# nolanderc/gpu-voxel-raytracer

Hardware: AMD Instinct MI355X
Metric: Mrays/s (higher is better)
Workload: dtype f32

## Files before the change

### gpu_voxel_raytracer_amd/csrc/api_context.hip

```cpp
#include <chrono>
#include <memory>

#include "ctx.h"

namespace vxrt {

size_t image_bytes(const vxrt_ctx* c) { return size_t(c->band.local_rows) * c->band.width * sizeof(float4); }
size_t display_bytes(const vxrt_ctx* c) { return size_t(c->band.local_rows) * c->band.width * 4u; }
bool is_display(vxrt_image which) { return which == VXRT_DISPLAY_BGRA8_SRGB || which == VXRT_DISPLAY_RGBA8_SRGB; }

int count_local_rows(const BandMap& b) {
    int rows = 0;
    for (int gb = b.rank; gb < band_count(b); gb += b.nranks) {
        const int y0 = band_first_row(b, gb), n = band_nominal_rows(b, gb);
        rows += (y0 + n <= b.height) ? n : b.height - y0;
    }
    return rows;
}

int local_band_count(const BandMap& b) {
    const int bands = band_count(b);
    return bands <= b.rank ? 0 : (bands - b.rank + b.nranks - 1) / b.nranks;
}

void free_images(vxrt_ctx* c) {
    c->ring.clear();
    c->ring_arena.reset();
    free_halo(c);
    for (DeviceBuf<float4>* p : {&c->accum[0], &c->accum[1], &c->denoised, &c->spp_sum}) p->reset();
    c->display.reset();
    c->schedules.clear();
    c->queues.clear();
    c->queue_bytes = 0;
    c->first_hits.clear();
}

int alloc_images(vxrt_ctx* c) {
    free_images(c);
    size_t bytes = image_bytes(c);
    if (bytes == 0) bytes = sizeof(float4);
    if (size_t(c->band.local_rows) * size_t(c->band.width) >= (size_t(1) << kPixBits)) {
        set_error("more than 2^27 pixels per context");
        return VXRT_E_INVALID;
    }
    c->ring.resize(size_t(c->inflight) * size_t(c->batch) + 2);
    const size_t pitch = (bytes + (size_t(2) << 20) - 1) & ~((size_t(2) << 20) - 1);
    HIP_TRY(c->ring_arena.alloc(pitch * 3 * c->ring.size()));
    HIP_TRY(hipMemsetAsync(c->ring_arena, 0, pitch * 3 * c->ring.size(), c->stream));
    size_t piece = 0;
// ... 36 lines not shown
                char* p = sq.rq_block;
                sq.rq.state[0] = reinterpret_cast<float4*>(p); p += kSegments * cap * 64;
                sq.rq.state[1] = reinterpret_cast<float4*>(p); p += kSegments * cap * 64;
                sq.rq.rays[0] = reinterpret_cast<float4*>(p); p += kSegments * cap * 64;
                sq.rq.rays[1] = reinterpret_cast<float4*>(p); p += kSegments * cap * 64;
                sq.rq.results[0] = reinterpret_cast<uint4*>(p); p += kSegments * cap * 32;
                sq.rq.results[1] = reinterpret_cast<uint4*>(p); p += kSegments * cap * 32;
                sq.rq.counts = reinterpret_cast<unsigned*>(p);
                sq.rq.seg_capacity = unsigned(cap);
            }
        }
    }
    if (c->batch >= 2 && c->band.local_rows > 0) {
        c->first_hits.resize(size_t(c->inflight));
        for (DeviceBuf<uint4>& p : c->first_hits) HIP_TRY(p.alloc(size_t(c->band.local_rows) * size_t(c->band.width)));
    }
    const size_t tiles = trace_tile_count(c->band.width, c->band.local_rows);
    c->schedules.resize(size_t(c->inflight));
    for (vxrt_ctx::TileSchedule& t : c->schedules) {
        for (DeviceBuf<uint32_t>* p : {&t.cost, &t.order, &t.last_cost}) {
            HIP_TRY(p->alloc(tiles + 1));
            HIP_TRY(hipMemsetAsync(p->get(), 0, (tiles + 1) * sizeof(uint32_t), c->stream));
        }
        HIP_TRY(t.scratch.alloc(256 * 128));
        if (c->trace_priority) {
            HIP_TRY(t.host_heavy.alloc(64 / sizeof(unsigned)));
            t.host_heavy[0] = 0u;
            HIP_TRY(t.heavy_ready.create(hipEventDisableTiming));
        }
    }
// ... 156 lines not shown
            return VXRT_OK;
        case VXRT_OPT_TAIL_CAPACITY:
            if (at_create) { c->tail_capacity_override = int(value > 0x7fffffffu ? 0x7fffffffu : value); return VXRT_OK; }
            if (c->trace_variant < 4) return VXRT_OK;
            c->tail_capacity_override = int(value > 0x7fffffffu ? 0x7fffffffu : value);
            return resize_tail_queues(c, value == 0 ? (c->shard_capacity_max / 8u < 4096u ? 4096u : c->shard_capacity_max / 8u) : value);
        case VXRT_OPT_SKY_CULL:
            if (value > 1) { set_error("sky cull must be 0 or 1"); return VXRT_E_INVALID; }
            c->sky_cull = int(value);
            return VXRT_OK;
        case VXRT_OPT_FRAME_LANES:
            if (value > 1) { set_error("frame lanes must be 0 or 1"); return VXRT_E_INVALID; }
            c->frame_lanes = int(value);
            return VXRT_OK;
        case VXRT_OPT_SHARED_PRIMARY:
            if (value > 1) { set_error("shared primary must be 0 or 1"); return VXRT_E_INVALID; }
            c->shared_primary = int(value);
            return VXRT_OK;
        case VXRT_OPT_HALO_ROWS:
            if (value > 4096) { set_error("halo rows must be 0..4096"); return VXRT_E_INVALID; }
            c->halo_min_rows = value;
            return VXRT_OK;
        case VXRT_OPT_TILE_ORDER:
            if (value > 1) { set_error("tile order must be 0 (raster) or 1 (longest first)"); return VXRT_E_INVALID; }
            c->use_tile_order = int(value);
            return VXRT_OK;
        case VXRT_OPT_TILE_SPREAD:
            if (value > 256 && value != VXRT_TILE_SPREAD_AUTO) { set_error("tile spread must be 0..256 or VXRT_TILE_SPREAD_AUTO"); return VXRT_E_INVALID; }
            c->spread_override = value == VXRT_TILE_SPREAD_AUTO ? -1 : int(value);
            return VXRT_OK;
        case VXRT_OPT_TRACE_BLOCKS:
// ... 443 lines not shown
    out->queue_overflow_paths = c->queue_overflow_paths;
    return VXRT_OK;
} VXRT_CATCH

int vxrt_reset_stats(vxrt_ctx* c) try {
    if (!valid_ctx(c)) return VXRT_E_INVALID;
    if (int rc = vxrt_sync(c)) return rc;
    HIP_TRY(hipMemsetAsync(c->d_rays, 0, kRaySlots * 64, c->stream));
    HIP_TRY(hipStreamSynchronize(c->stream));
    c->frames = c->pixels = c->timed_frames = c->timed_launches = 0;
    c->queue_overflow_paths = 0;
    c->ms[0] = c->ms[1] = c->ms[2] = c->ms[3] = c->ms[4] = 0.0;
    c->halo_exchanges = 0;
    c->frame_lane_launches = 0;
    c->shared_primary_launches = 0;
    c->split_launches = 0;
    return VXRT_OK;
} VXRT_CATCH


}
```

### gpu_voxel_raytracer_amd/csrc/api_debug.hip

```cpp
#include "../../include/vxrt_bluenoise.h"
#include "ctx.h"

extern "C" {

int vxrt_debug_tile_costs(vxrt_ctx* c, uint32_t* out, size_t n) try {
    if (!valid_ctx(c) || !out) { set_error("null argument"); return VXRT_E_INVALID; }
    const size_t out_x = size_t((c->band.width + 15) / 16), out_y = size_t((c->band.local_rows + 15) / 16);
    if (n != out_x * out_y || c->schedules.empty()) { set_error("tile count mismatch"); return VXRT_E_INVALID; }
    HIP_TRY(hipSetDevice(c->cfg.device));
    if (int rc = sync_all(c)) return rc;
    int tw = 16, th = 16;
    trace_tile_dims(&tw, &th);
    const size_t kx = size_t((c->band.width + tw - 1) / tw), ky = size_t((c->band.local_rows + th - 1) / th);
    std::vector<uint32_t> raw(kx * ky);
    HIP_TRY(hipMemcpy(raw.data(), c->schedules[size_t(c->last_schedule)].last_cost, raw.size() * sizeof(uint32_t), hipMemcpyDeviceToHost));
    for (size_t i = 0; i < n; i++) out[i] = 0;
    for (size_t y = 0; y < ky; y++)
        for (size_t x = 0; x < kx; x++) {
            uint32_t& o = out[(y * size_t(th) / 16) * out_x + x * size_t(tw) / 16];
            o = raw[y * kx + x] > o ? raw[y * kx + x] : o;
        }
    return VXRT_OK;
} VXRT_CATCH

// ... 117 lines not shown
    return VXRT_OK;
} VXRT_CATCH

int vxrt_debug_culled_pixels(vxrt_ctx* c, uint64_t* count) try {
    if (!valid_ctx(c) || !count) { set_error("null argument"); return VXRT_E_INVALID; }
    if (!c->has_scene) { set_error("no scene set"); return VXRT_E_NOSCENE; }
    HIP_TRY(hipSetDevice(c->cfg.device));
    if (int rc = vxrt_sync(c)) return rc;
    const Cam keep_cam = c->cam, keep_old = c->old_cam;
    const vxrt_uniforms keep_u = c->uniforms;
    update_bindings(c);
    TraceArgs a{};
    frame_constants(c, a);
    a.cam = c->cam;
    a.batch = 1;
    set_cull(c, a, &a.cam, 1);
    c->cam = keep_cam; c->old_cam = keep_old; c->uniforms = keep_u;
    ScratchBuffer b;
    HIP_TRY(b.alloc(sizeof(unsigned long long)));
    HIP_TRY(hipMemsetAsync(b.as<unsigned long long>(), 0, sizeof(unsigned long long), c->stream));
    HIP_TRY(launch_count_culled(a, b.as<unsigned long long>(), c->stream));
    HIP_TRY(hipStreamSynchronize(c->stream));
    unsigned long long n = 0;
    HIP_TRY(hipMemcpy(&n, b.as<unsigned long long>(), sizeof n, hipMemcpyDeviceToHost));
    *count = n;
    return VXRT_OK;
} VXRT_CATCH

int vxrt_debug_shared_primary_launches(vxrt_ctx* c, uint64_t* count) try {
    if (!valid_ctx(c) || !count) { set_error("null argument"); return VXRT_E_INVALID; }
    *count = c->shared_primary_launches;
    return VXRT_OK;
} VXRT_CATCH

int vxrt_debug_dda_rays(vxrt_ctx* c, const float* origins, const float* dirs, size_t n, uint32_t flags, float margin_scale, uint32_t max_steps,
                        float* out_walk, float* out_dda, double ms[4]) try {
    if (!valid_ctx(c) || !origins || !dirs || !out_dda || !ms || (!out_walk && !(flags & 4u))) { set_error("null argument"); return VXRT_E_INVALID; }
#if !VXRT_VARIANTS
    set_error("the DDA prototype is not in this build of libvxrt (compile with -DVXRT_VARIANTS=1)");
    return VXRT_E_INVALID;
#else
    if (!c->has_scene) { set_error("no scene set"); return VXRT_E_NOSCENE; }
    const int levels = int(c->depth) + 1;
    if (levels < 3 || levels > 12) { set_error("the DDA grid wants a tree of depth 2..11 (4 .. 4096 cells per axis)"); return VXRT_E_INVALID; }
    if (n == 0) return VXRT_OK;
    HIP_TRY(hipSetDevice(c->cfg.device));
// ... 176 lines not shown
```

### gpu_voxel_raytracer_amd/csrc/api_frame.hip

```cpp
#include "ctx.h"

namespace vxrt {

int check_render(vxrt_ctx* c, uint32_t flags) {
    if (!valid_ctx(c)) return VXRT_E_INVALID;
    const uint32_t stages = VXRT_ALL | VXRT_DENOISE_INTERIOR | VXRT_DENOISE_EDGE;
    if ((flags & stages) == 0) { set_error("no stage selected"); return VXRT_E_INVALID; }
    if ((flags & VXRT_DENOISE) && (flags & (VXRT_DENOISE_INTERIOR | VXRT_DENOISE_EDGE))) {
        set_error("VXRT_DENOISE is the whole stage: it does not combine with VXRT_DENOISE_INTERIOR / VXRT_DENOISE_EDGE");
        return VXRT_E_INVALID;
    }
    if (!c->has_scene) { set_error("vxrt_render before any scene was set"); return VXRT_E_NOSCENE; }
    const bool window = c->band.nranks > 1 && c->denoise.radius > 0;
    const bool any_denoise = (flags & (VXRT_DENOISE | VXRT_DENOISE_INTERIOR | VXRT_DENOISE_EDGE)) != 0;
    const bool reads_halo = (flags & (VXRT_DENOISE | VXRT_DENOISE_EDGE)) != 0;
    if (any_denoise && window && c->band.band_rows % 16 != 0) {
        set_error("denoise with radius > 0 on row bands needs band_rows to be a multiple of 16 (its 16x16 tiles must not straddle bands)");
        return VXRT_E_INVALID;
    }
    if (reads_halo && window && (flags & (VXRT_TRACE | VXRT_TEMPORAL))) {
        set_error("multi-rank denoise with radius > 0 needs the halo: render TRACE|TEMPORAL, exchange, then DENOISE (or DENOISE_INTERIOR "
                  "while the messages travel and DENOISE_EDGE after vxrt_halo_unpack)");
        return VXRT_E_INVALID;
    }
// ... 101 lines not shown
    if (post) {
        HIP_TRY(hipEventRecord(cur.own, c->stream));
        cur.last_use = cur.own;
        cur.last_use_recorded = true;
    }
    return VXRT_OK;
}

}

extern "C" {

int vxrt_render(vxrt_ctx* c, uint32_t flags) try {
    if (int rc = check_render(c, flags)) return rc;
    HIP_TRY(hipSetDevice(c->cfg.device));
    const bool timed = (flags & VXRT_TIMED) != 0;
    if (flags & VXRT_TRACE) {
        int slot = 0;
        Cam cam, old;
        if (int rc = trace_frames(c, 1, timed, &slot, &cam, &old)) return rc;
    }
    if (int rc = post_stages(c, flags, timed)) return rc;
    if (flags & VXRT_TRACE) c->old_cam_valid = true;
    return VXRT_OK;
} VXRT_CATCH

static int render_sequence(vxrt_ctx* c, uint32_t flags, uint32_t count, const float (*path_pos)[3], const float (*path_dir)[3]) {
    const bool timed = (flags & VXRT_TIMED) != 0;
    const uint32_t batch = (flags & VXRT_TRACE) && batches_frames(c->trace_variant) ? uint32_t(c->batch) : 1u;
    if (batch <= 1) {
// ... 14 lines not shown
        for (uint32_t k = 0; k < g; k++) {
            c->slot = slots[k];
            c->cam = cams[k];
            c->old_cam = olds[k];
            if (int rc = post_stages(c, flags, timed)) return rc;
            c->old_cam_valid = true;
        }
        done += g;
    }
    return VXRT_OK;
}

int vxrt_render_frames(vxrt_ctx* c, uint32_t flags, uint32_t count) try {
    if (int rc = check_render(c, flags)) return rc;
    HIP_TRY(hipSetDevice(c->cfg.device));
    return render_sequence(c, flags, count, nullptr, nullptr);
} VXRT_CATCH

int vxrt_render_path(vxrt_ctx* c, uint32_t flags, uint32_t count, const float (*positions)[3], const float (*directions)[3], float fov) try {
    if (int rc = check_render(c, flags)) return rc;
    if (!positions || !directions) { set_error("null argument"); return VXRT_E_INVALID; }
    HIP_TRY(hipSetDevice(c->cfg.device));
    c->cam_fov = fov;
    return render_sequence(c, flags, count, positions, directions);
} VXRT_CATCH

int vxrt_render_spp(vxrt_ctx* c, uint32_t flags, uint32_t spp) try {
    if (int rc = check_render(c, flags)) return rc;
    if (!(flags & VXRT_TRACE) || spp == 0 || spp > 4096) { set_error("vxrt_render_spp needs VXRT_TRACE and 1 <= spp <= 4096"); return VXRT_E_INVALID; }
    HIP_TRY(hipSetDevice(c->cfg.device));
    const bool timed = (flags & VXRT_TIMED) != 0;
    const size_t pixels = size_t(c->band.local_rows) * c->band.width;
    if (spp > 1 && c->spp_sum == nullptr && pixels > 0) HIP_TRY(c->spp_sum.alloc(pixels));
    const uint32_t batch = batches_frames(c->trace_variant) ? uint32_t(c->batch) : 1u;
    Cam first_old{};
    for (uint32_t done = 0; done < spp;) {
        const uint32_t g = spp - done < batch ? spp - done : batch;
        int slots[kMaxBatch];
        Cam cams[kMaxBatch], olds[kMaxBatch];
        const uint32_t gbuf = done + g == spp ? 1u << (g - 1u) : 0u;
        if (int rc = trace_frames(c, g, timed, slots, cams, olds, nullptr, nullptr, gbuf)) return rc;
        if (done == 0) first_old = olds[0];
        if (spp > 1 && pixels > 0) {
            SppArgs a{};
            for (uint32_t k = 0; k < g; k++) {
// ... 30 lines not shown
```

### gpu_voxel_raytracer_amd/csrc/api_trace.hip

```cpp
#include <algorithm>
#include <cmath>

#include "ctx.h"
#include "vx_vec.h"

namespace vxrt {

int resize_tail_queues(vxrt_ctx* c, unsigned want) {
    want = want > c->shard_capacity_max ? c->shard_capacity_max : (want + 63u) / 64u * 64u;
    if (want == c->shard_capacity) return VXRT_OK;
    if (int rc = sync_all(c)) return rc;
    const size_t new_bytes = (size_t(want) * 64 + 1) * 64, old_bytes = (size_t(c->shard_capacity) * 64 + 1) * 64;
    std::vector<DeviceBuf<float4>> fresh;
    for (vxrt_ctx::StreamQueues& q : c->queues)
        for (DeviceBuf<float4>& p : q.hitq)
            if (p) {
                fresh.emplace_back();
                if (hipError_t e = fresh.back().alloc(new_bytes / sizeof(float4)); e != hipSuccess) return hip_fail(e, "hipMalloc (tail queues)");
            }
    size_t k = 0;
    for (vxrt_ctx::StreamQueues& q : c->queues)
        for (DeviceBuf<float4>& p : q.hitq)
            if (p) {
                p.swap(fresh[k++]);
// ... 62 lines not shown
#endif
    f3 sun_dir = mk3(vx_cos(u.sun_yaw) * vx_cos(u.sun_pitch), -vx_sin(u.sun_pitch), vx_sin(u.sun_yaw) * vx_cos(u.sun_pitch));
    f3 sun_n = norm3(sun_dir), neg_sun_n = norm3(-sun_dir);
    f3 sun_color = u.sun_strength * mk3(u.sun_color[0], u.sun_color[1], u.sun_color[2]);
    a.sun_dir[0] = sun_dir.x; a.sun_dir[1] = sun_dir.y; a.sun_dir[2] = sun_dir.z;
    a.sun_dir_n[0] = sun_n.x; a.sun_dir_n[1] = sun_n.y; a.sun_dir_n[2] = sun_n.z;
    a.neg_sun_dir_n[0] = neg_sun_n.x; a.neg_sun_dir_n[1] = neg_sun_n.y; a.neg_sun_dir_n[2] = neg_sun_n.z;
    a.sun_color[0] = sun_color.x; a.sun_color[1] = sun_color.y; a.sun_color[2] = sun_color.z;
    a.sky_color[0] = u.sky_color[0]; a.sky_color[1] = u.sky_color[1]; a.sky_color[2] = u.sky_color[2];
    a.sun_exponent = 1.0f / (u.sun_size * u.sun_size);
    a.sun_zero_below = 0.0f;
    if (a.sun_exponent > 1.0f && a.sun_exponent < 1e6f) a.sun_zero_below = float(exp(-88.0 / double(a.sun_exponent)) * (1.0 - 1e-4));
    a.sun_size = u.sun_size; a.sun_strength = u.sun_strength; a.emit_strength = u.emit_strength; a.specularity = u.specularity;
}

void set_cull(const vxrt_ctx* c, TraceArgs& a, const Cam* cams, uint32_t g) {
    a.cull = 0;
    if (c->sky_cull && c->box_valid) {
        float far = 0.0f;
        bool sane = true;
        for (uint32_t k = 0; k < g; k++)
            for (int i = 0; i < 3; i++) {
                const float v = fabsf(cams[k].o[i]);
                sane = sane && v < 1e6f && std::isfinite(cams[k].r[i]) && std::isfinite(cams[k].u[i]) && std::isfinite(cams[k].f[i]);
                far = v > far ? v : far;
            }
        if (sane) {
            const float m = 0.01f + ldexpf(far + 2.0f * c->root_size, -16);
            for (int i = 0; i < 3; i++) { a.cull_min[i] = c->box_min[i] - m; a.cull_max[i] = c->box_max[i] + m; }
            a.cull = 1;
        }
    }
}

static int xcd_affine_order(vxrt_ctx* c, vxrt_ctx::TileSchedule& sched, hipStream_t ts) {
    const unsigned tiles = trace_tile_count(c->band.width, c->band.local_rows);
    int tw = 8, th = 8;
    trace_tile_dims(&tw, &th);
    const unsigned tx = unsigned(c->band.width + tw - 1) / unsigned(tw), ty = tiles / (tx ? tx : 1u);
    const unsigned S = unsigned(c->xcd_affinity);
    std::vector<uint32_t> cost(tiles), order;
    order.reserve(tiles);
    HIP_TRY(hipStreamSynchronize(ts));
    HIP_TRY(hipMemcpy(cost.data(), sched.cost, size_t(tiles) * 4, hipMemcpyDeviceToHost));
    const unsigned sx = (tx + S - 1) / S, sy = (ty + S - 1) / S;
    std::vector<unsigned long long> scost(size_t(sx) * sy, 0ull);
    for (unsigned t = 0; t < tiles; t++)
// ... 42 lines not shown
}


struct CountSets {
    unsigned* sets[3] = {nullptr, nullptr, nullptr};
    unsigned J = 0;
    CountSets() = default;
    explicit CountSets(const vxrt_ctx::StreamQueues& sq) : sets{sq.counts3, sq.counts3 + 64 * 16, sq.counts3 + 2 * 64 * 16}, J(sq.launches) {}
    unsigned* read() const { return sets[J % 3]; }
    unsigned* written() const { return sets[(J + 1) % 3]; }
    unsigned* cleared() const { return sets[(J + 2) % 3]; }
};

struct TraceLaunch {
    vxrt_ctx* c; hipStream_t ts; size_t lane; uint32_t g; const int* slots;
    TracePlan plan{};
    TraceArgs a;
    CountSets counts;
    TraceLaunch(vxrt_ctx* c_, hipStream_t ts_, size_t lane_, uint32_t g_, const int* slots_) : c(c_), ts(ts_), lane(lane_), g(g_), slots(slots_) {}
};

static float path_motion_px(const vxrt_ctx* c, uint32_t g, uint32_t F, const float (*path_pos)[3], const float (*path_dir)[3]) {
    const float f_px = 0.5f * float(c->cfg.height) / tanf(0.5f * c->cam_fov);
    float worst = 0.0f;
    for (uint32_t k = 0; k + F <= g; k += F) {
        const float* p0 = path_pos[k]; const float* p1 = path_pos[k + F - 1];
        const float* d0 = path_dir[k]; const float* d1 = path_dir[k + F - 1];
        const float n0 = sqrtf(d0[0] * d0[0] + d0[1] * d0[1] + d0[2] * d0[2]), n1 = sqrtf(d1[0] * d1[0] + d1[1] * d1[1] + d1[2] * d1[2]);
        float cosang = (d0[0] * d1[0] + d0[1] * d1[1] + d0[2] * d1[2]) / (n0 * n1);
        cosang = cosang > 1.0f ? 1.0f : (cosang < -1.0f ? -1.0f : cosang);
        const float ang = acosf(cosang);
        const float dp = sqrtf((p1[0] - p0[0]) * (p1[0] - p0[0]) + (p1[1] - p0[1]) * (p1[1] - p0[1]) + (p1[2] - p0[2]) * (p1[2] - p0[2]));
        float dist = sqrtf((p0[0] - c->root_center[0]) * (p0[0] - c->root_center[0]) + (p0[1] - c->root_center[1]) * (p0[1] - c->root_center[1]) +
                           (p0[2] - c->root_center[2]) * (p0[2] - c->root_center[2]));
        dist = dist < 0.05f * c->root_size ? 0.05f * c->root_size : dist;
        const float px = f_px * (ang > dp / dist ? ang : dp / dist);
        worst = !(px <= worst) ? px : worst;
    }
    return worst;
}

static void plan_trace(TracePlan& p, const vxrt_ctx* c, uint32_t g, const Cam* cams, const float (*path_pos)[3], const float (*path_dir)[3], size_t lane) {
    const bool wide = use_wide(c);
    const vxrt_ctx::TileSchedule& sched = c->schedules[lane];
    const bool ordered = c->use_tile_order && sched.valid;
    const unsigned tiles = trace_tile_count(c->band.width, c->band.local_rows);
    p.hbm = c->svo_count * sizeof(SvoRecord) + c->leaf_count * sizeof(int32_t) > kInfinityCacheBytes;
    p.tracer = (c->auto_tracer && (p.hbm || (g == 1 && c->inflight == 1))) ? 0 : c->trace_variant;
    p.wide_head = wide && (p.tracer == 0 || p.tracer == 4);
    p.wide_tail = wide;
    p.single_tail_launch = p.tracer == 4;
    for (int k = c->tail_from + 1; p.single_tail_launch && k < int(c->cfg.max_bounces); k++)
        if (c->queues[lane].hitq[1] && ((c->tail_split >> k) & 1u)) p.single_tail_launch = false;
    const bool fused = c->fused_tail && p.single_tail_launch && !wide && !p.hbm && c->tail_from < int(c->cfg.max_bounces);
    p.path = p.tracer == 0 ? TracePath::all_in_one : p.tracer == 2 ? TracePath::wavefront : p.tracer < 4 ? TracePath::ray_queue :
             fused ? TracePath::fused : p.tracer == 5 ? TracePath::head_paths : TracePath::head_bounces;
    const bool trace_kernel_head = p.path == TracePath::all_in_one || p.path == TracePath::head_bounces || p.path == TracePath::head_paths;
    p.frame_lanes = (c->frame_lanes && !wide && !p.hbm) ? (g % 8u == 0u ? 8 : (g % 4u == 0u ? 4 : 0)) : 0;
    if (p.frame_lanes && path_pos != nullptr && !(path_motion_px(c, g, uint32_t(p.frame_lanes), path_pos, path_dir) <= 16.0f)) p.frame_lanes = 0;
    p.share = trace_kernel_head && c->shared_primary && g >= 2 && lane < c->first_hits.size() && c->first_hits[lane] != nullptr && !wide && !p.hbm;
    for (uint32_t k = 1; p.share && k < g; k++) p.share = memcmp(&cams[k], &cams[0], sizeof(Cam)) == 0;
    if (p.path == TracePath::head_bounces && c->long_tiles_permille > 0 && ordered && p.tracer == 4 && !wide && !p.hbm) {
        const unsigned n = unsigned((unsigned long long)tiles * c->long_tiles_permille / 1000u);
        p.long_blocks = (n < 1u ? 1u : (n >= tiles ? tiles - 1u : n)) * g;
    }
    if (trace_kernel_head && c->trace_priority && ordered && !sched.heavy_pending && p.long_blocks == 0u && sched.heavy < tiles) p.split_heavy = sched.heavy;
    if (batches_frames(p.tracer) && c->use_tile_order && (!sched.valid || sched.age >= 8))
        p.sort = (c->xcd_affinity > 0 && g == 1 && p.hbm) ? TileSort::xcd_affine : TileSort::longest_first;
}

static void next_frames(vxrt_ctx* c, uint32_t g, int* slots, Cam* cams, Cam* olds, const float (*path_pos)[3], const float (*path_dir)[3]) {
    for (uint32_t k = 0; k < g; k++) {
        if (path_pos) {
            memcpy(c->cam_pos, path_pos[k], sizeof c->cam_pos);
            memcpy(c->cam_dir, path_dir[k], sizeof c->cam_dir);
        }
// ... 34 lines not shown
static void fill_trace_args(TraceLaunch& L, const Cam* cams, uint32_t gbuf_frames, uint32_t first_frame_number) {
    const vxrt_ctx* c = L.c;
    TraceArgs& a = L.a;
    const uint32_t g = L.g;
    const vxrt_ctx::TileSchedule& sched = c->schedules[L.lane];
    frame_constants(c, a);
    for (uint32_t k = 0; k < g; k++) {
        const vxrt_ctx::Slot& sl = c->ring[size_t(L.slots[k])];
        a.out[k] = FrameOut{sl.sampled_color, sl.nd, sl.albedo};
        a.cams[k] = cams[k];
    }
    a.out_color = a.out[0].color; a.out_nd = a.out[0].nd; a.out_albedo = a.out[0].albedo;
    a.batch = int(g);
    a.gbuf_frames = gbuf_frames;
    a.frame_lanes = L.plan.frame_lanes;
    set_cull(c, a, cams, g);
    a.ray_counter = c->d_rays;
    a.tile_order = (c->use_tile_order && sched.valid) ? sched.order : nullptr;
    a.tile_cost = c->use_tile_order ? sched.cost : nullptr;
    a.frame_number = first_frame_number;
    a.cam = cams[0];
    a.tail = PathQueue{nullptr, nullptr, 0};
    a.tail_zero = nullptr;
    a.tail_from = 0;
    if (L.plan.tracer != 0) L.counts = CountSets(c->queues[L.lane]);
    if (L.plan.tracer >= 4) {
        a.tail = PathQueue{c->queues[L.lane].hitq[0], L.counts.written(), c->shard_capacity};
        a.tail_zero = L.counts.cleared();
        a.tail_from = c->tail_from;
    }
}
// ... 32 lines not shown
        HIP_TRY(c->aux_streams[lane].create(hipStreamNonBlocking));
        HIP_TRY(c->aux_fork[lane].create(hipEventDisableTiming));
        HIP_TRY(c->aux_join[lane].create(hipEventDisableTiming));
    }
    TraceArgs al = L.a;
    al.tail = PathQueue{nullptr, nullptr, 0};
    al.tail_zero = nullptr;
    HIP_TRY(hipEventRecord(c->aux_fork[lane], L.ts));
    HIP_TRY(hipStreamWaitEvent(c->aux_streams[lane], c->aux_fork[lane], 0));
    HIP_TRY(launch_trace(al, false, false, c->aux_streams[lane], 0u, L.plan.long_blocks));
    HIP_TRY(hipEventRecord(c->aux_join[lane], c->aux_streams[lane]));
    return VXRT_OK;
}

static int issue_head(TraceLaunch& L) {
    if (L.plan.long_blocks != 0u) { if (int rc = fork_long_tiles(L)) return rc; }
    if (L.plan.share) {
        L.a.first_hit = L.c->first_hits[L.lane];
        HIP_TRY(launch_first_hit(L.a, L.ts));
    }
    return issue_trace_kernel(L);
}

static int tail_bounces(TraceLaunch& L) {
    vxrt_ctx* c = L.c;
    vxrt_ctx::StreamQueues& sq = c->queues[L.lane];
    PathQueue queues[2] = {{sq.hitq[0], nullptr, c->shard_capacity}, {sq.hitq[1], nullptr, sq.hitq[1] ? c->shard_capacity : 0u}};
    HIP_TRY(launch_bounces(L.a, L.plan.wide_tail, queues, L.counts.sets, &sq.launches, c->trace_blocks, sq.hitq[1] ? c->tail_split : 0u, c->tail_from, L.ts));
    return VXRT_OK;
}

#if VXRT_VARIANTS
static int tail_paths(TraceLaunch& L) {
    HIP_TRY(launch_paths(L.a, L.a.tail, L.counts.read(), L.c->tail_from, L.c->path_blocks, L.ts));
// ... 105 lines not shown
        vxrt_ctx::Slot& sl = c->ring[size_t(L.slots[k])];
        sl.trace_done = done;
        sl.last_use = done;
        sl.last_use_recorded = true;
    }
    c->slot = L.slots[g - 1];
    c->last_schedule = int(lane);
    c->trace_launches += 1;
    c->traced += g;
    c->frames += g;
    c->pixels += uint64_t(g) * uint64_t(c->band.local_rows) * c->band.width;
    if (timed) { c->timed_frames += g; c->timed_launches += 1; }
    c->accum_is_sampled = true;
    c->halo_valid = false;
    if (L.plan.frame_lanes) c->frame_lane_launches++;
    if (L.plan.share) c->shared_primary_launches++;
    if (L.plan.split_heavy) c->split_launches++;
    return VXRT_OK;
}

int trace_frames(vxrt_ctx* c, uint32_t g, bool timed, int* slots, Cam* cams, Cam* olds, const float (*path_pos)[3], const float (*path_dir)[3],
                 uint32_t gbuf_frames) {
    const uint32_t first_frame_number = c->uniforms.frame_number + 1;
    next_frames(c, g, slots, cams, olds, path_pos, path_dir);
    const size_t lane = size_t(c->trace_launches % uint64_t(c->inflight));
    hipStream_t ts = c->trace_streams[lane];
    if (int rc = wait_for_slots(c, g, slots, ts)) return rc;
    TraceLaunch L(c, ts, lane, g, slots);
    if (c->band.local_rows > 0) {
        if (int rc = absorb_feedback(c, lane)) return rc;
        plan_trace(L.plan, c, g, cams, path_pos, path_dir, lane);
        fill_trace_args(L, cams, gbuf_frames, first_frame_number);
        EventPair p;
        if (timed) { p = take_pair(c, 0); HIP_TRY(hipEventRecord(p.a, ts)); }
        if (int rc = issue(L)) return rc;
        if (c->trace_priority && batches_frames(L.plan.tracer)) HIP_TRY(hipStreamWaitEvent(ts, c->low_join[lane], 0));
        if (timed) HIP_TRY(hipEventRecord(p.b, ts));
        if (int rc = resort_tiles(L)) return rc;
        if (timed) c->pending.push_back(p);
    }
    return finish_launch(L, timed);
}

}
```

### gpu_voxel_raytracer_amd/csrc/ctx.h

```cpp
#pragma once
#include <hip/hip_runtime.h>

#include <cstdint>
#include <cstdlib>
#include <cstring>
#include <new>
#include <stdexcept>
#include <string>
#include <vector>

#include "../../include/vxrt.h"
#include "../../include/vxrt_debug.h"
#include "../../include/vxrt_host.h"
#include "kernels.h"
#include "owned.h"
#include "scene_host.h"

namespace vxrt {
const std::string& last_error();

constexpr size_t kNoiseCount = size_t(512) * 128 * 128;

inline int hip_fail(hipError_t e, const char* what) {
    set_error(std::string(what) + ": " + hipGetErrorString(e));
// ... 30 lines not shown
    if (direct) {
        HIP_TRY(write(static_cast<int16_t*>(pos), static_cast<uint32_t*>(mrgb)));
        return VXRT_OK;
    }
    if (int rc = alloc_scratch(&stage[0], count * 3 * sizeof(int16_t), who, "the positions")) return rc;
    if (int rc = alloc_scratch(&stage[1], count * 4, who, "the mrgb words")) return rc;
    HIP_TRY(write(stage[0].as<int16_t>(), stage[1].as<uint32_t>()));
    HIP_TRY(hipMemcpyAsync(pos, stage[0].get(), count * 3 * sizeof(int16_t), hipMemcpyDeviceToDevice, s));
    HIP_TRY(hipMemcpyAsync(mrgb, stage[1].get(), count * 4, hipMemcpyDeviceToDevice, s));
    return VXRT_OK;
}

struct EventPair {
    hipEvent_t a = nullptr, b = nullptr;
    int stage = 0;
};
}

using namespace vxrt;

struct vxrt_ctx {
    vxrt_config cfg{};
    BandMap band{};
    Stream stream;
    std::vector<Stream> own_trace_streams;
    std::vector<hipStream_t> trace_streams;
    std::vector<Stream> aux_streams;
    std::vector<Stream> low_streams;
    Stream copy_stream;

// ... 115 lines not shown
        Event heavy_ready;
        bool heavy_pending = false;
        unsigned heavy = 0;
    };
    std::vector<TileSchedule> schedules;
    int last_schedule = 0;
    int use_tile_order = 1;
    int trace_blocks = 2048;
    int spread_override = -1;
    int node_order = 0;
    int node_order_applied = 0;
    int host_scene_build = 0;
    unsigned wave_slots = 5120;
    int frame_lanes = 1;
    uint32_t frame_lane_launches = 0;
    int shared_primary = 1;
    uint64_t shared_primary_launches = 0;
    std::vector<DeviceBuf<uint4>> first_hits;
    int path_blocks = 512;
    int tail_from = 1;
    unsigned tail_split = 0;
    unsigned trace_split = 0x1;
    uint64_t frames = 0, pixels = 0, timed_frames = 0;
    double ms[5] = {0, 0, 0, 0, 0};
    uint64_t halo_exchanges = 0;
    std::vector<EventPair> pending, free_pairs;
    std::vector<Event> pair_events;

    struct ReadSlot {
        DeviceBuf<char> stage;
        size_t stage_bytes = 0;
        Event snap, arrived;
        bool in_flight = false;
// ... 16 lines not shown
    int dda_levels = 0;
};

namespace vxrt {
constexpr size_t kInfinityCacheBytes = size_t(256) << 20;
inline bool batches_frames(int tracer) { return tracer == 0 || tracer >= 4; }
enum class TracePath { all_in_one, head_bounces, head_paths, fused, wavefront, ray_queue };
enum class TileSort { none, longest_first, xcd_affine };
struct TracePlan {
    bool hbm;
    bool wide_head, wide_tail;
    int tracer;
    TracePath path;
    int frame_lanes;
    bool share;
    unsigned long_blocks;
    bool single_tail_launch;
    unsigned split_heavy;
    TileSort sort;
};

inline void drop_dda_grid(vxrt_ctx* c) {
    for (DeviceBuf<void>& g : c->dda_grid) g.reset();
    c->dda_levels = 0;
}
inline void drop_touch_maps(vxrt_ctx* c) {
    c->d_touch_nodes.reset();
    c->d_touch_leaves.reset();
    c->touch_node_lines = c->touch_leaf_lines = 0;
    drop_dda_grid(c);
// ... 15 lines not shown
bool valid_ctx(const vxrt_ctx* c);
float4* image_ptr(vxrt_ctx* c, vxrt_image which);
bool is_display(vxrt_image which);
size_t display_bytes(const vxrt_ctx* c);
bool use_wide(const vxrt_ctx* c);
bool scene_box(const SvoRecord* recs, size_t count, uint32_t depth, const float root_center[3], float root_size, float box_min[3], float box_max[3]);
int device_scene_box(const SvoRecord* svo, size_t nsvo, uint32_t depth, SvoRecord root, const float root_center[3], float root_size, bool* valid,
                     float box_min[3], float box_max[3]);
void replace_scene_arrays(vxrt_ctx* c, DeviceBuf<SvoRecord>&& svo, size_t nsvo, DeviceBuf<int32_t>&& leaves, size_t nleaves, DeviceBuf<WideRec>&& wide,
                          size_t nwide);
int install_scene(vxrt_ctx* c, DeviceBuf<SvoRecord>&& svo, size_t nsvo, DeviceBuf<int32_t>&& lw, size_t nlw, uint32_t depth, SvoRecord root,
                  DeviceBuf<WideRec>&& wide, size_t nwide, WideRec wide_root);
int widen_svo(const std::vector<SvoRecord>& recs, uint32_t depth, std::vector<WideRec>* out);
int resize_tail_queues(vxrt_ctx* c, unsigned want);
int apply_option(vxrt_ctx* c, uint32_t option, uint32_t value, bool at_create);
void set_cull(const vxrt_ctx* c, TraceArgs& a, const Cam* cams, uint32_t g);
int grow_tail_queues(vxrt_ctx* c, size_t lane);
void update_bindings(vxrt_ctx* c);
void frame_constants(const vxrt_ctx* c, TraceArgs& a);
int trace_frames(vxrt_ctx* c, uint32_t g, bool timed, int* slots, Cam* cams, Cam* olds, const float (*path_pos)[3] = nullptr,
                 const float (*path_dir)[3] = nullptr, uint32_t gbuf_frames = 0xffffffffu);
int check_render(vxrt_ctx* c, uint32_t flags);
int post_stages(vxrt_ctx* c, uint32_t flags, bool timed);
void free_halo(vxrt_ctx* c);
int build_tile_rows(vxrt_ctx* c);
uint32_t halo_rows_wanted(const vxrt_ctx* c);
}
```

### gpu_voxel_raytracer_amd/host.py

```python
import contextlib
import ctypes as C
import os


import numpy as np

from . import _build

_LIB = None


class VxrtError(RuntimeError):
    def __init__(self, status, where, detail=""):
        self.status = status
        self.detail = detail
        super().__init__(f"{where}: status {status} ({detail})")


OK, E_INVALID, E_DEVICE = 0, -1, -2
E_VOX_MAGIC, E_VOX_VERSION, E_VOX_NOMAIN, E_VOX_EOF, E_VOX_CHUNK = -10, -11, -12, -13, -14
E_VOX_MATERIAL, E_VOX_NOMATL, E_VOX_NOMODEL, E_IO, E_SCENE, E_NOSCENE, E_NOISE = -15, -16, -17, -18, -20, -21, -30

GRID_PALETTE8, GRID_WORD32 = 1, 2
SOLID_UNION, SOLID_INTERIOR = 0, 1
# ... 1274 lines not shown

    def render_stage(self, flags):
        self._chk(self._L.vxrt_render(self._h, C.c_uint32(flags)), "vxrt_render")

    def culled_pixels(self):
        n = C.c_uint64(0)
        self.update_bindings()
        self._chk(self._L.vxrt_debug_culled_pixels(self._h, C.byref(n)), "vxrt_debug_culled_pixels")
        return int(n.value)

    def shared_primary_launches(self):
        n = C.c_uint64(0)
        self._chk(self._L.vxrt_debug_shared_primary_launches(self._h, C.byref(n)), "vxrt_debug_shared_primary_launches")
        return int(n.value)

    def set_option(self, option, value):
        self._chk(self._L.vxrt_set_option(self._h, C.c_int(option), C.c_uint32(value)), "vxrt_set_option")

    def sync(self):
        self._chk(self._L.vxrt_sync(self._h), "vxrt_sync")

    def reset_history(self):
        self._chk(self._L.vxrt_reset_history(self._h), "vxrt_reset_history")

    def set_frame_number(self, n):
        self._chk(self._L.vxrt_set_frame_number(self._h, C.c_uint32(n)), "vxrt_set_frame_number")

    def local_rows(self):
        n = C.c_uint32(0)
        self._chk(self._L.vxrt_local_rows(self._h, C.byref(n), None), "vxrt_local_rows")
# ... 90 lines not shown
```

### include/vxrt_debug.h

```cpp
#ifndef VXRT_DEBUG_H
#define VXRT_DEBUG_H

#include "vxrt.h"

#ifdef __cplusplus
extern "C" {
#endif

#define VXRT_OPT_TILE_ORDER ((vxrt_option)7)
#define VXRT_OPT_TILE_SPREAD ((vxrt_option)8)
#define VXRT_OPT_TRACE_BLOCKS ((vxrt_option)9)
#define VXRT_OPT_TAIL_FROM ((vxrt_option)10)
#define VXRT_OPT_TAIL_SPLIT ((vxrt_option)11)
#define VXRT_OPT_HOST_SCENE_BUILD ((vxrt_option)12)
#define VXRT_OPT_TRACER_OVERRIDE ((vxrt_option)13)
#define VXRT_OPT_TRACE_SPLIT ((vxrt_option)14)
#define VXRT_OPT_PATH_BLOCKS ((vxrt_option)15)
#define VXRT_OPT_SHADE_BLOCKS ((vxrt_option)16)
#define VXRT_OPT_RAYS_PER_WAVE ((vxrt_option)17)
#define VXRT_OPT_NODE_ORDER ((vxrt_option)18)
#define VXRT_OPT_HEAD_STAGGER ((vxrt_option)19)
#define VXRT_OPT_LONG_TILES ((vxrt_option)20)
#define VXRT_OPT_FUSED_TAIL ((vxrt_option)21)
#define VXRT_OPT_TRACE_PRIORITY ((vxrt_option)22)
// ... 16 lines not shown

int vxrt_display_thresholds(float out[255]);
int vxrt_debug_display_encode(int32_t device, const float* rgba, size_t n_pixels, uint32_t format, uint8_t* out);

int vxrt_debug_cast_rays(vxrt_ctx* ctx, const float* origins, const float* dirs, size_t n, uint8_t* hit, float* time, int32_t* node,
                         float* normal);

int vxrt_debug_path_log(vxrt_ctx* ctx, int32_t x, int32_t y, float* log, int32_t* casts);

int vxrt_debug_tile_costs(vxrt_ctx* ctx, uint32_t* out, size_t n);

int vxrt_debug_tile_order(vxrt_ctx* ctx, uint32_t* order, uint32_t* cost, size_t n, uint32_t* walking_tiles, uint32_t* spread_256);

int vxrt_debug_culled_pixels(vxrt_ctx* ctx, uint64_t* count);
int vxrt_debug_shared_primary_launches(vxrt_ctx* ctx, uint64_t* count);
int vxrt_debug_fused_profile(vxrt_ctx* ctx, uint64_t out[8]);

int vxrt_debug_touch_map(vxrt_ctx* ctx, uint32_t enable);
int vxrt_debug_touch_count(vxrt_ctx* ctx, uint64_t out[6], uint32_t reset);

int vxrt_debug_dda_rays(vxrt_ctx* ctx, const float* origins, const float* dirs, size_t n, uint32_t flags, float margin_scale, uint32_t max_steps,
                        float* out_walk, float* out_dda, double ms[4]);

int vxrt_debug_morph_tile_lookup(vxrt_ctx* ctx, uint32_t enable);

enum { VXRT_FEATURE_VARIANTS = 1 };
uint32_t vxrt_build_features(void);

#ifdef __cplusplus
}
// ... 3 lines not shown
```

Measured before the change: 32710.

## Reuse primary first-hit buffer across launches within one render call

Adds shared-primary mode 2, now the default, which tags a first-hit buffer with the call id, camera and cull box. Later trace launches in the same render call with a matching camera and cull box reuse that buffer instead of re-walking the primary rays. Cross-stream events order the work: reusing lanes wait on the walk event, and a new walk waits for earlier readers of its buffer. This removes repeated primary-ray traversal, at the cost of extra inter-stream dependencies that can reduce overlap between in-flight lanes.

```diff
diff --git a/gpu_voxel_raytracer_amd/csrc/api_context.hip b/gpu_voxel_raytracer_amd/csrc/api_context.hip
--- a/gpu_voxel_raytracer_amd/csrc/api_context.hip
+++ b/gpu_voxel_raytracer_amd/csrc/api_context.hip
@@ -33,6 +33,9 @@
     c->queues.clear();
     c->queue_bytes = 0;
     c->first_hits.clear();
+    c->first_hit_walked.clear();
+    c->first_hit_readers.clear();
+    c->first_hit_tag = vxrt_ctx::FirstHitTag{};
 }
 
 int alloc_images(vxrt_ctx* c) {
@@ -99,6 +102,9 @@
     if (c->batch >= 2 && c->band.local_rows > 0) {
         c->first_hits.resize(size_t(c->inflight));
         for (DeviceBuf<uint4>& p : c->first_hits) HIP_TRY(p.alloc(size_t(c->band.local_rows) * size_t(c->band.width)));
+        c->first_hit_walked.resize(size_t(c->inflight));
+        for (Event& e : c->first_hit_walked) HIP_TRY(e.create(hipEventDisableTiming));
+        c->first_hit_readers.assign(size_t(c->inflight) * size_t(c->inflight), nullptr);
     }
     const size_t tiles = trace_tile_count(c->band.width, c->band.local_rows);
     c->schedules.resize(size_t(c->inflight));
@@ -285,7 +291,7 @@
             c->frame_lanes = int(value);
             return VXRT_OK;
         case VXRT_OPT_SHARED_PRIMARY:
-            if (value > 1) { set_error("shared primary must be 0 or 1"); return VXRT_E_INVALID; }
+            if (value > 2) { set_error("shared primary must be 0 (off), 1 (one walk per launch) or 2 (one walk per call)"); return VXRT_E_INVALID; }
             c->shared_primary = int(value);
             return VXRT_OK;
         case VXRT_OPT_HALO_ROWS:
@@ -759,6 +765,7 @@
     c->halo_exchanges = 0;
     c->frame_lane_launches = 0;
     c->shared_primary_launches = 0;
+    c->first_hit_walks = 0;
     c->split_launches = 0;
     return VXRT_OK;
 } VXRT_CATCH
diff --git a/gpu_voxel_raytracer_amd/csrc/api_debug.hip b/gpu_voxel_raytracer_amd/csrc/api_debug.hip
--- a/gpu_voxel_raytracer_amd/csrc/api_debug.hip
+++ b/gpu_voxel_raytracer_amd/csrc/api_debug.hip
@@ -155,7 +155,7 @@
     frame_constants(c, a);
     a.cam = c->cam;
     a.batch = 1;
-    set_cull(c, a, &a.cam, 1);
+    set_cull(a, cull_box(c, &a.cam, 1));
     c->cam = keep_cam; c->old_cam = keep_old; c->uniforms = keep_u;
     ScratchBuffer b;
     HIP_TRY(b.alloc(sizeof(unsigned long long)));
@@ -171,6 +171,12 @@
 int vxrt_debug_shared_primary_launches(vxrt_ctx* c, uint64_t* count) try {
     if (!valid_ctx(c) || !count) { set_error("null argument"); return VXRT_E_INVALID; }
     *count = c->shared_primary_launches;
+    return VXRT_OK;
+} VXRT_CATCH
+
+int vxrt_debug_first_hit_walks(vxrt_ctx* c, uint64_t* count) try {
+    if (!valid_ctx(c) || !count) { set_error("null argument"); return VXRT_E_INVALID; }
+    *count = c->first_hit_walks;
     return VXRT_OK;
 } VXRT_CATCH
 
diff --git a/gpu_voxel_raytracer_amd/csrc/api_frame.hip b/gpu_voxel_raytracer_amd/csrc/api_frame.hip
--- a/gpu_voxel_raytracer_amd/csrc/api_frame.hip
+++ b/gpu_voxel_raytracer_amd/csrc/api_frame.hip
@@ -139,6 +139,7 @@
 int vxrt_render(vxrt_ctx* c, uint32_t flags) try {
     if (int rc = check_render(c, flags)) return rc;
     HIP_TRY(hipSetDevice(c->cfg.device));
+    c->call_id++;
     const bool timed = (flags & VXRT_TIMED) != 0;
     if (flags & VXRT_TRACE) {
         int slot = 0;
@@ -183,6 +184,7 @@
 int vxrt_render_frames(vxrt_ctx* c, uint32_t flags, uint32_t count) try {
     if (int rc = check_render(c, flags)) return rc;
     HIP_TRY(hipSetDevice(c->cfg.device));
+    c->call_id++;
     return render_sequence(c, flags, count, nullptr, nullptr);
 } VXRT_CATCH
 
@@ -190,6 +192,7 @@
     if (int rc = check_render(c, flags)) return rc;
     if (!positions || !directions) { set_error("null argument"); return VXRT_E_INVALID; }
     HIP_TRY(hipSetDevice(c->cfg.device));
+    c->call_id++;
     c->cam_fov = fov;
     return render_sequence(c, flags, count, positions, directions);
 } VXRT_CATCH
@@ -198,6 +201,7 @@
     if (int rc = check_render(c, flags)) return rc;
     if (!(flags & VXRT_TRACE) || spp == 0 || spp > 4096) { set_error("vxrt_render_spp needs VXRT_TRACE and 1 <= spp <= 4096"); return VXRT_E_INVALID; }
     HIP_TRY(hipSetDevice(c->cfg.device));
+    c->call_id++;
     const bool timed = (flags & VXRT_TIMED) != 0;
     const size_t pixels = size_t(c->band.local_rows) * c->band.width;
     if (spp > 1 && c->spp_sum == nullptr && pixels > 0) HIP_TRY(c->spp_sum.alloc(pixels));
diff --git a/gpu_voxel_raytracer_amd/csrc/api_trace.hip b/gpu_voxel_raytracer_amd/csrc/api_trace.hip
--- a/gpu_voxel_raytracer_amd/csrc/api_trace.hip
+++ b/gpu_voxel_raytracer_amd/csrc/api_trace.hip
@@ -100,8 +100,8 @@
     a.sun_size = u.sun_size; a.sun_strength = u.sun_strength; a.emit_strength = u.emit_strength; a.specularity = u.specularity;
 }
 
-void set_cull(const vxrt_ctx* c, TraceArgs& a, const Cam* cams, uint32_t g) {
-    a.cull = 0;
+CullBox cull_box(const vxrt_ctx* c, const Cam* cams, uint32_t g) {
+    CullBox b;
     if (c->sky_cull && c->box_valid) {
         float far = 0.0f;
         bool sane = true;
@@ -113,10 +113,16 @@
             }
         if (sane) {
             const float m = 0.01f + ldexpf(far + 2.0f * c->root_size, -16);
-            for (int i = 0; i < 3; i++) { a.cull_min[i] = c->box_min[i] - m; a.cull_max[i] = c->box_max[i] + m; }
-            a.cull = 1;
+            for (int i = 0; i < 3; i++) { b.lo[i] = c->box_min[i] - m; b.hi[i] = c->box_max[i] + m; }
+            b.on = 1;
         }
     }
+    return b;
+}
+
+void set_cull(TraceArgs& a, const CullBox& b) {
+    a.cull = b.on;
+    for (int i = 0; i < 3; i++) { a.cull_min[i] = b.lo[i]; a.cull_max[i] = b.hi[i]; }
 }
 
 static int xcd_affine_order(vxrt_ctx* c, vxrt_ctx::TileSchedule& sched, hipStream_t ts) {
@@ -189,6 +195,7 @@
 
 struct TraceLaunch {
     vxrt_ctx* c; hipStream_t ts; size_t lane; uint32_t g; const int* slots;
+    CullBox cull{};
     TracePlan plan{};
     TraceArgs a;
     CountSets counts;
@@ -215,7 +222,8 @@
     return worst;
 }
 
-static void plan_trace(TracePlan& p, const vxrt_ctx* c, uint32_t g, const Cam* cams, const float (*path_pos)[3], const float (*path_dir)[3], size_t lane) {
+static void plan_trace(TracePlan& p, const vxrt_ctx* c, uint32_t g, const Cam* cams, const CullBox& cull, const float (*path_pos)[3], const float (*path_dir)[3],
+                       size_t lane) {
     const bool wide = use_wide(c);
     const vxrt_ctx::TileSchedule& sched = c->schedules[lane];
     const bool ordered = c->use_tile_order && sched.valid;
@@ -235,6 +243,14 @@
     if (p.frame_lanes && path_pos != nullptr && !(path_motion_px(c, g, uint32_t(p.frame_lanes), path_pos, path_dir) <= 16.0f)) p.frame_lanes = 0;
     p.share = trace_kernel_head && c->shared_primary && g >= 2 && lane < c->first_hits.size() && c->first_hits[lane] != nullptr && !wide && !p.hbm;
     for (uint32_t k = 1; p.share && k < g; k++) p.share = memcmp(&cams[k], &cams[0], sizeof(Cam)) == 0;
+    p.walk = p.share;
+    p.hits = lane;
+    const vxrt_ctx::FirstHitTag& tag = c->first_hit_tag;
+    if (p.share && c->shared_primary == 2 && tag.call != 0 && tag.call == c->call_id && tag.buffer < c->first_hits.size() &&
+        memcmp(&tag.cam, &cams[0], sizeof(Cam)) == 0 && tag.cull == cull) {
+        p.walk = false;
+        p.hits = tag.buffer;
+    }
     if (p.path == TracePath::head_bounces && c->long_tiles_permille > 0 && ordered && p.tracer == 4 && !wide && !p.hbm) {
         const unsigned n = unsigned((unsigned long long)tiles * c->long_tiles_permille / 1000u);
         p.long_blocks = (n < 1u ? 1u : (n >= tiles ? tiles - 1u : n)) * g;
@@ -299,7 +315,7 @@
     a.batch = int(g);
     a.gbuf_frames = gbuf_frames;
     a.frame_lanes = L.plan.frame_lanes;
-    set_cull(c, a, cams, g);
+    set_cull(a, L.cull);
     a.ray_counter = c->d_rays;
     a.tile_order = (c->use_tile_order && sched.valid) ? sched.order : nullptr;
     a.tile_cost = c->use_tile_order ? sched.cost : nullptr;
@@ -362,10 +378,30 @@
 }
 
 static int issue_head(TraceLaunch& L) {
+    vxrt_ctx* c = L.c;
     if (L.plan.long_blocks != 0u) { if (int rc = fork_long_tiles(L)) return rc; }
     if (L.plan.share) {
-        L.a.first_hit = L.c->first_hits[L.lane];
-        HIP_TRY(launch_first_hit(L.a, L.ts));
+        const size_t b = L.plan.hits, streams = c->trace_streams.size();
+        vxrt_ctx::FirstHitTag& tag = c->first_hit_tag;
+        L.a.first_hit = c->first_hits[b];
+        if (L.plan.walk) {
+            for (size_t s = 0; s < streams; s++) {
+                hipEvent_t& reader = c->first_hit_readers[b * streams + s];
+                if (reader != nullptr && s != L.lane) HIP_TRY(hipStreamWaitEvent(L.ts, reader, 0));
+                reader = nullptr;
+            }
+            tag.call = 0;
+            HIP_TRY(launch_first_hit(L.a, L.ts));
+            if (c->shared_primary == 2) {
+                HIP_TRY(hipEventRecord(c->first_hit_walked[b], L.ts));
+                tag.call = c->call_id;
+                tag.buffer = b;
+                tag.cam = L.a.cams[0];
+                tag.cull = L.cull;
+            }
+        } else if (b != L.lane) {
+            HIP_TRY(hipStreamWaitEvent(L.ts, c->first_hit_walked[b], 0));
+        }
     }
     return issue_trace_kernel(L);
 }
@@ -501,7 +537,11 @@
     c->accum_is_sampled = true;
     c->halo_valid = false;
     if (L.plan.frame_lanes) c->frame_lane_launches++;
-    if (L.plan.share) c->shared_primary_launches++;
+    if (L.plan.share) {
+        c->shared_primary_launches++;
+        c->first_hit_readers[L.plan.hits * c->trace_streams.size() + lane] = done;
+    }
+    if (L.plan.walk) c->first_hit_walks++;
     if (L.plan.split_heavy) c->split_launches++;
     return VXRT_OK;
 }
@@ -516,7 +556,8 @@
     TraceLaunch L(c, ts, lane, g, slots);
     if (c->band.local_rows > 0) {
         if (int rc = absorb_feedback(c, lane)) return rc;
-        plan_trace(L.plan, c, g, cams, path_pos, path_dir, lane);
+        L.cull = cull_box(c, cams, g);
+        plan_trace(L.plan, c, g, cams, L.cull, path_pos, path_dir, lane);
         fill_trace_args(L, cams, gbuf_frames, first_frame_number);
         EventPair p;
         if (timed) { p = take_pair(c, 0); HIP_TRY(hipEventRecord(p.a, ts)); }
diff --git a/gpu_voxel_raytracer_amd/csrc/ctx.h b/gpu_voxel_raytracer_amd/csrc/ctx.h
--- a/gpu_voxel_raytracer_amd/csrc/ctx.h
+++ b/gpu_voxel_raytracer_amd/csrc/ctx.h
@@ -68,6 +68,12 @@
 struct EventPair {
     hipEvent_t a = nullptr, b = nullptr;
     int stage = 0;
+};
+
+struct CullBox {
+    int on = 0;
+    float lo[3] = {0, 0, 0}, hi[3] = {0, 0, 0};
+    bool operator==(const CullBox& o) const { return on == o.on && (on == 0 || (memcmp(lo, o.lo, sizeof lo) == 0 && memcmp(hi, o.hi, sizeof hi) == 0)); }
 };
 }
 
@@ -213,9 +219,20 @@
     unsigned wave_slots = 5120;
     int frame_lanes = 1;
     uint32_t frame_lane_launches = 0;
-    int shared_primary = 1;
+    int shared_primary = 2;
     uint64_t shared_primary_launches = 0;
+    uint64_t first_hit_walks = 0;
     std::vector<DeviceBuf<uint4>> first_hits;
+    std::vector<Event> first_hit_walked;
+    std::vector<hipEvent_t> first_hit_readers;
+    uint64_t call_id = 0;
+    struct FirstHitTag {
+        uint64_t call = 0;
+        size_t buffer = 0;
+        Cam cam{};
+        CullBox cull{};
+    };
+    FirstHitTag first_hit_tag;
     int path_blocks = 512;
     int tail_from = 1;
     unsigned tail_split = 0;
@@ -262,6 +279,8 @@
     TracePath path;
     int frame_lanes;
     bool share;
+    bool walk;
+    size_t hits;
     unsigned long_blocks;
     bool single_tail_launch;
     unsigned split_heavy;
@@ -307,7 +326,8 @@
 int widen_svo(const std::vector<SvoRecord>& recs, uint32_t depth, std::vector<WideRec>* out);
 int resize_tail_queues(vxrt_ctx* c, unsigned want);
 int apply_option(vxrt_ctx* c, uint32_t option, uint32_t value, bool at_create);
-void set_cull(const vxrt_ctx* c, TraceArgs& a, const Cam* cams, uint32_t g);
+CullBox cull_box(const vxrt_ctx* c, const Cam* cams, uint32_t g);
+void set_cull(TraceArgs& a, const CullBox& b);
 int grow_tail_queues(vxrt_ctx* c, size_t lane);
 void update_bindings(vxrt_ctx* c);
 void frame_constants(const vxrt_ctx* c, TraceArgs& a);
diff --git a/gpu_voxel_raytracer_amd/host.py b/gpu_voxel_raytracer_amd/host.py
--- a/gpu_voxel_raytracer_amd/host.py
+++ b/gpu_voxel_raytracer_amd/host.py
@@ -1312,6 +1312,11 @@
         self._chk(self._L.vxrt_debug_shared_primary_launches(self._h, C.byref(n)), "vxrt_debug_shared_primary_launches")
         return int(n.value)
 
+    def first_hit_walks(self):
+        n = C.c_uint64(0)
+        self._chk(self._L.vxrt_debug_first_hit_walks(self._h, C.byref(n)), "vxrt_debug_first_hit_walks")
+        return int(n.value)
+
     def set_option(self, option, value):
         self._chk(self._L.vxrt_set_option(self._h, C.c_int(option), C.c_uint32(value)), "vxrt_set_option")
 
diff --git a/include/vxrt_debug.h b/include/vxrt_debug.h
--- a/include/vxrt_debug.h
+++ b/include/vxrt_debug.h
@@ -54,6 +54,7 @@
 
 int vxrt_debug_culled_pixels(vxrt_ctx* ctx, uint64_t* count);
 int vxrt_debug_shared_primary_launches(vxrt_ctx* ctx, uint64_t* count);
+int vxrt_debug_first_hit_walks(vxrt_ctx* ctx, uint64_t* count);
 int vxrt_debug_fused_profile(vxrt_ctx* ctx, uint64_t out[8]);
 
 int vxrt_debug_touch_map(vxrt_ctx* ctx, uint32_t enable);
```

Result: faster. 33680 (median of 6 runs) (+2.9%).
